# JoshuaQSH/FALCON-TTDforGNNs

Measured on AMD Instinct MI355X. Metric: tt_embedding_lookups_per_sec, higher is better.
Workload: dtype f32; 1 GPU; ogbn-products TTEmbeddingBag fwd+bwd+SGD per step, frontier of a 2048-seed batch = 409600 unique uniform ids per GPU, bag length 1; num_embeddings=2449029, ids_per_gpu_step=409600, parallelism=dp1

## Files before the change

### falcon-ttdforgnns_amd/csrc/ttemb_fast3.hip

```cpp
#include "ttemb_common.h"
#include "ttemb_cache.h"

#include <atomic>
#include <cstdlib>
#include <cstring>



namespace ttemb {

typedef float f32x4 __attribute__((ext_vector_type(4)));


constexpr int kChunk = 16;
constexpr uint32_t kMultiBit = 0x80000000u;

template <int Q0, int Q1, int Q2, int R1, int R2>
struct Cfg {
  static constexpr int M2 = Q0 * Q1;
  static constexpr int MT2 = (M2 + 15) / 16;
  static constexpr int KS1 = R1 / 4;
  static constexpr int KS2 = R2 / 4;
  static constexpr int N1 = Q1 * R2;
  static constexpr int NT1 = (N1 + 15) / 16;
  static constexpr int NT2 = Q2;
  static constexpr int D = Q0 * Q1 * Q2;
  static constexpr int ROW0 = Q0 * R1;
  static constexpr int ROW1 = R1 * Q1 * R2;
  static constexpr int ROW2 = R2 * Q2;
  static constexpr int LDA = R2 + 1;
  static constexpr int LDB = ROW2 + 4;
  static constexpr int LDO = D + 4;
  static constexpr int P_FLOATS = ((MT2 * 16 * LDA + 3) / 4) * 4;
  static constexpr int B_FLOATS = kChunk * LDB;
  static constexpr int O_FLOATS = kChunk * LDO;
  static constexpr int LDPB = (R2 % 32 == 0) ? R2 + 16 : R2;
  static constexpr int LDBB = (Q2 % 2 == 1 && ROW2 % 32 == 16) ? ROW2 : ROW2 + 4;
  static constexpr int BB2_FLOATS = kChunk * LDBB;
  static constexpr int DPAD = (M2 + 3) / 4 * 4 * Q2;
  static constexpr int LDOB = (((DPAD > D ? DPAD : D) + 15) / 32) * 32 + 16;
  static constexpr int OB_FLOATS = kChunk * LDOB;
  static constexpr int PB_FLOATS = ((M2 * LDPB + 3) / 4) * 4;
  static constexpr int BO_FLOATS = B_FLOATS > O_FLOATS ? B_FLOATS : O_FLOATS;
  static constexpr int WAVE_FLOATS = P_FLOATS + BO_FLOATS;
  static constexpr int RT1 = (R1 + 15) / 16;
  static constexpr int RT2 = (R2 + 15) / 16;
  static constexpr int LDG = N1 + 1;
  static constexpr int LD2 = ROW2 + 1;
  static constexpr int BB_FLOATS = B_FLOATS > P_FLOATS ? B_FLOATS : P_FLOATS;
  static constexpr int DB_FLOATS = ((O_FLOATS > R1 * LDG ? O_FLOATS : R1 * LDG) + 3) / 4 * 4;
  static constexpr int BWD_WAVE_FLOATS = P_FLOATS + BB_FLOATS + DB_FLOATS;
  static_assert(LDOB >= (M2 + 3) / 4 * 4 * Q2, "the padded K-step of the E product reads inside the staged row");
  static_assert(Q0 <= 16, "stage 1 pads q0 to one 16-row tile");
  static_assert(R1 % 4 == 0 && R2 % 4 == 0, "ranks must be multiples of the MFMA K");
  static_assert(N1 % 4 == 0, "rows of the prefix product move as float4");
  static_assert(D % 4 == 0 && ROW2 % 4 == 0, "rows move as float4");
  static_assert(ROW2 <= 256, "the dG2 reduce reads one E row per wavefront load");
};

typedef unsigned int u32x4 __attribute__((ext_vector_type(4)));
typedef __amdgpu_buffer_rsrc_t rsrc_t;
constexpr uint32_t kOob = 0xffffffffu;

__device__ __forceinline__ rsrc_t make_rsrc(const void* p, uint32_t bytes) {
  return __builtin_amdgcn_make_buffer_rsrc(const_cast<void*>(p), 0, (int)bytes, 0x00020000);
}
__device__ __forceinline__ float4 buf_load4(rsrc_t r, uint32_t voff) {
  const u32x4 v = __builtin_amdgcn_raw_buffer_load_b128(r, (int)voff, 0, 0);
  return make_float4(__uint_as_float(v.x), __uint_as_float(v.y), __uint_as_float(v.z), __uint_as_float(v.w));
}
__device__ __forceinline__ u32x4 buf_load4u(rsrc_t r, uint32_t voff) {
  return __builtin_amdgcn_raw_buffer_load_b128(r, (int)voff, 0, 0);
}
__device__ __forceinline__ uint32_t buf_load1u(rsrc_t r, uint32_t voff) {
  return __builtin_amdgcn_raw_buffer_load_b32(r, (int)voff, 0, 0);
}
__device__ __forceinline__ void buf_store4(rsrc_t r, uint32_t voff, const float4& x) {
  u32x4 v;
  v.x = __float_as_uint(x.x);
  v.y = __float_as_uint(x.y);
  v.z = __float_as_uint(x.z);
  v.w = __float_as_uint(x.w);
  __builtin_amdgcn_raw_buffer_store_b128(v, r, (int)voff, 0, 0);
}
#ifndef TTEMB_NT
#define TTEMB_NT 0
#endif
template <bool NT>
__device__ __forceinline__ void buf_store4_p(rsrc_t r, uint32_t voff, const float4& x) {
  u32x4 v;
  v.x = __float_as_uint(x.x);
  v.y = __float_as_uint(x.y);
  v.z = __float_as_uint(x.z);
  v.w = __float_as_uint(x.w);
  __builtin_amdgcn_raw_buffer_store_b128(v, r, (int)voff, 0, NT ? 2 : 0);
}
__device__ __forceinline__ void buf_store1(rsrc_t r, uint32_t voff, float x) {
  __builtin_amdgcn_raw_buffer_store_b32(__float_as_uint(x), r, (int)voff, 0, 0);
}

typedef const __attribute__((address_space(4))) uint32_t* desc_ptr;
__device__ __forceinline__ uint4 load_desc(desc_ptr tab, uint32_t c, uint32_t nchunks) {
  const uint32_t at = 4u * (c < nchunks ? c : (nchunks ? nchunks - 1 : 0u));
  const uint32_t keep = c < nchunks ? 0xffffffffu : 0u;
  return make_uint4(tab[at] & keep, tab[at + 1] & keep, tab[at + 2] & keep, tab[at + 3] & keep);
}

constexpr int kSortThreads = 1024;
#ifndef TTEMB_RANGE_THREADS
#define TTEMB_RANGE_THREADS 512
#endif
constexpr int kRangeThreads = TTEMB_RANGE_THREADS;
#ifndef TTEMB_SORT_SLICE
#define TTEMB_SORT_SLICE 2048
#endif
constexpr int kSliceIds = TTEMB_SORT_SLICE;
constexpr int kMaxSlices = 1024;
constexpr int kMaxRanges = 512;
constexpr int kSortBatch = 8;
constexpr uint32_t kFirstBit = 0x100u, kLastBit = 0x200u;
constexpr int kCountBanks = 8;
__host__ __device__ __forceinline__ uint64_t counter_tag(uint64_t epoch) { return ((epoch & ((1ull << 37) - 1ull)) | (1ull << 37)) << 26; }
constexpr int kOvfBits = 28;
constexpr uint64_t kOvfMask = (1ull << kOvfBits) - 1ull;
__host__ __device__ __forceinline__ uint64_t ovf_tag(uint64_t epoch) { return ((epoch & ((1ull << 35) - 1ull)) | (1ull << 35)) << kOvfBits; }
constexpr uint32_t kNoGroup = 0xffffffffu;
constexpr uint32_t kNoBlock = 0xffffffffu;
constexpr int kRoundIds = kSortThreads * 4;

struct Piece {
  long long pos0;
  long long count;
  long long rowbase;
  long long zero0, zero1;
  long long window_bytes;
};

struct GroupPlan {
  const Piece* piece;
  uint2* bucket;
  uint2* ovf;
  uint64_t* ovf_count;
  uint64_t* ovf_head;
  uint32_t cap;
  uint32_t banks;
  uint32_t ovf_slots;
  uint64_t* rcount;
  uint32_t* gstamp;
  uint64_t* epochs;
  uint64_t* rpub;
  uint32_t* i2s;
  uint32_t* vals;
  uint32_t* counts;
  uint64_t* gpre;
  uint4* ctab;
  float* ptab;
  float* etab;
  float* dptab;
  float* g2part;
  float* g0part;
  float* g1part;
  uint32_t* epi_live;
  uint32_t* wrows;
  uint32_t* wnrows;
  uint32_t* ticket;
  uint32_t use_ticket;
  uint32_t* fault_host;
  uint32_t spin_limit;
  uint32_t keep_p;
};

constexpr uint32_t kFaultTakeOver = 1u, kFaultLookBack = 2u, kFaultOverflow = 3u;
__device__ __forceinline__ uint64_t plan_tag(const GroupPlan& plan, uint64_t call) {
  const uint64_t salt = (reinterpret_cast<uint64_t>(plan.epochs) >> 8) * 0x9e3779b97f4a7c15ull;
  return (((call + salt) & ((1ull << 39) - 1ull)) | (1ull << 39)) << 24;
}
__device__ __forceinline__ void report_fault(const GroupPlan& plan, uint32_t G, uint64_t call, uint32_t code) {
  __hip_atomic_store(&plan.gpre[G + 2u], plan_tag(plan, call) | code, __ATOMIC_RELAXED, __HIP_MEMORY_SCOPE_AGENT);
  if (plan.fault_host != nullptr) __hip_atomic_store(plan.fault_host, code, __ATOMIC_RELAXED, __HIP_MEMORY_SCOPE_SYSTEM);
}
__device__ __forceinline__ bool plan_poisoned(const GroupPlan& plan, uint32_t G) {
  const desc_ptr w = (desc_ptr)plan.gpre;
  const uint32_t t_lo = w[2u * G + 2u], t_hi = w[2u * G + 3u], f_lo = w[2u * G + 4u], f_hi = w[2u * G + 5u];
  return t_hi == f_hi && ((t_lo ^ f_lo) >> 24) == 0u && (t_hi >> 31) != 0u;
}

__device__ __forceinline__ void poison_output(const GroupPlan& plan, float* out, uint32_t out_bytes, uint32_t row_floats, uint32_t gw,
                                              uint32_t nwaves, int lane) {
  if (plan.piece != nullptr) {
    out += plan.piece->rowbase * (long long)row_floats;
    out_bytes = (uint32_t)plan.piece->window_bytes;
  }
  const rsrc_t r = __builtin_amdgcn_make_buffer_rsrc(out, 0, (int)out_bytes, 0x00020000);
  const uint32_t qnan = 0x7fc00000u;
  u32x4 v;
  v.x = v.y = v.z = v.w = qnan;
  for (uint64_t off = ((uint64_t)gw * 64u + (uint32_t)lane) * 16u; off < out_bytes; off += (uint64_t)nwaves * 1024u)
    __builtin_amdgcn_raw_buffer_store_b128(v, r, (int)(uint32_t)off, 0, 0);
}

__device__ __forceinline__ uint64_t pack_count(uint32_t c) {
  return (uint64_t)c | ((uint64_t)((c + kChunk - 1) / kChunk) << 32);
}

template <typename T, int NT>
__device__ __forceinline__ T block_exclusive(T v, T* wave_sums, T& total) {
  const int lane = threadIdx.x & 63, wave = threadIdx.x >> 6;
  T incl = v;
#pragma unroll
  for (int d = 1; d < kWave; d <<= 1) {
    T up;
    if constexpr (sizeof(T) == 8) {
      const uint32_t lo_w = __shfl_up((uint32_t)incl, d, kWave), hi_w = __shfl_up((uint32_t)((uint64_t)incl >> 32), d, kWave);
      up = (T)((uint64_t)lo_w | ((uint64_t)hi_w << 32));
    } else {
      up = __shfl_up(incl, d, kWave);
    }
    if (lane >= d) incl += up;
  }
  if (lane == kWave - 1) wave_sums[wave] = incl;
  __syncthreads();
  T before = 0, all = 0;
  for (int w = 0; w < NT / kWave; ++w) {
    const T x = wave_sums[w];
    if (w < wave) before += x;
    all += x;
  }
  __syncthreads();
  total = all;
  return before + incl - v;
}

__device__ __forceinline__ uint64_t tagged_add(uint64_t* word, uint64_t tag, uint64_t mask, uint64_t v, uint32_t spin_limit,
                                               bool& taken) {
  unsigned long long* ctr = reinterpret_cast<unsigned long long*>(word);
  unsigned long long old = atomicAdd(ctr, (unsigned long long)v);
  taken = true;
  if ((old & ~mask) == tag) return old & mask;
  for (uint32_t tries = 0; tries < spin_limit; ++tries) {
    old = __hip_atomic_load(ctr, __ATOMIC_RELAXED, __HIP_MEMORY_SCOPE_AGENT);
    if ((old & ~mask) == tag) return atomicAdd(ctr, (unsigned long long)v) & mask;
    if (atomicCAS(ctr, old, tag | v) == old) return 0;
  }
  taken = false;
  return 0;
}

__global__ __launch_bounds__(kSortThreads) void fast3_decode_kernel(
    const int64_t* __restrict__ indices, const int64_t* __restrict__ rowidx,
    const int64_t* __restrict__ offsets, uint32_t nnz, uint32_t per_slice,
    const int32_t* __restrict__ nnz_dev, int64_t B, int D, float* __restrict__ zero_out, uint32_t sentinel,
    uint32_t p0, uint32_t p1, uint32_t p2, uint32_t shift, uint32_t ranges, GroupPlan plan) {
  __shared__ uint32_t hist[kMaxRanges];
  __shared__ uint32_t place[kMaxRanges];
  __shared__ uint32_t oslot[kMaxRanges];
  const uint64_t call = plan.epochs[0] + 1ull;
  const uint32_t epoch = (uint32_t)call;
  if (blockIdx.x == 0 && threadIdx.x == 0) {
    plan.epochs[1] = call;
    *plan.ticket = 0u;
  }
  const Piece* pc = plan.piece;
  const int64_t pos0 = pc ? pc->pos0 : 0, rowbase = pc ? pc->rowbase : 0;
  const int64_t cnt = pc ? pc->count : live_count(nnz, nnz_dev);
  const int64_t cnt_all = pos0 + cnt;
  const uint32_t s0 = blockIdx.x * per_slice;
  if (zero_out != nullptr) {
    const int64_t z0 = pc ? pc->zero0 : 0, z1 = pc ? pc->zero1 : B;
    const int64_t per_b = (z1 - z0 + gridDim.x - 1) / gridDim.x;
    const int64_t b1 = z0 + (blockIdx.x + 1) * per_b < z1 ? z0 + (blockIdx.x + 1) * per_b : z1;
    for (int64_t b = z0 + blockIdx.x * per_b + threadIdx.x; b < b1; b += kSortThreads)
      if (offsets[b + 1] - offsets[b] != 1) {
        float4* o = reinterpret_cast<float4*>(zero_out + b * D);
        for (int c = 0; c * 4 < D; ++c) o[c] = make_float4(0.f, 0.f, 0.f, 0.f);
      }
  }
  const uint32_t s1 = s0 + per_slice < nnz ? s0 + per_slice : nnz;
  const uint32_t bank = blockIdx.x % plan.banks, cap = plan.cap;
  const uint64_t tag = counter_tag(call), otag = ovf_tag(call);
  uint64_t* const rctr = plan.rcount + (size_t)bank * kMaxRanges;
  uint2* const bkt = plan.bucket + (size_t)bank * cap;
  const size_t rstride = (size_t)plan.banks * cap;
  constexpr int UD = kRoundIds / kSortThreads;
  for (uint32_t r0 = s0; r0 < s1; r0 += kRoundIds) {
    for (uint32_t i = threadIdx.x; i < ranges; i += kSortThreads) hist[i] = 0u;
    __syncthreads();
    int64_t idv[UD], o0[UD], o1[UD], rv[UD];
#pragma unroll
    for (int u = 0; u < UD; ++u) {
      const uint32_t n = r0 + threadIdx.x + u * kSortThreads;
      const int64_t g = pos0 + n;
      const bool on = n < s1 && (int64_t)n < cnt;
      idv[u] = on ? indices[g] : 0;
      rv[u] = on && rowidx != nullptr ? rowidx[g] : -1;
      const bool direct = on && rowidx == nullptr && g < B;
      o0[u] = direct ? offsets[g] : -1;
      o1[u] = direct ? offsets[g + 1] : -1;
    }
    uint32_t key[UD], val[UD], rng[UD], rank[UD];
#pragma unroll
    for (int u = 0; u < UD; ++u) {
      const uint32_t n = r0 + threadIdx.x + u * kSortThreads;
      rng[u] = kNoGroup;
      key[u] = val[u] = rank[u] = 0u;
      if (n >= s1 || (int64_t)n >= cnt) continue;
      int64_t id = idv[u];
      id = id < 0 ? 0 : (id >= (int64_t)sentinel ? (int64_t)sentinel - 1 : id);
      const int64_t g = pos0 + n;
      int64_t row;
      bool multi;
      if (rowidx != nullptr) {
        row = rv[u];
        multi = !bag_is_single(rowidx, offsets, g, cnt_all, row);
      } else if (o0[u] >= 0 && o0[u] <= g && g < o1[u]) {
        row = g;
        multi = o1[u] - o0[u] != 1;
      } else {
        int64_t lo = 0, hi = B;
        while (hi - lo > 1) {
          const int64_t mid = (lo + hi) >> 1;
          if (offsets[mid] <= g) lo = mid; else hi = mid;
        }
        row = lo;
        multi = offsets[row + 1] - offsets[row] != 1;
      }
      row -= rowbase;
      const uint32_t uu = (uint32_t)id;
      const uint32_t i0 = uu / (p1 * p2);
      const uint32_t rem = uu - i0 * (p1 * p2);
      const uint32_t i1 = rem / p2;
      const uint32_t group = i1 * p0 + i0;
      key[u] = (group & ((1u << shift) - 1u)) | ((rem - i1 * p2) << 16);
      val[u] = (uint32_t)row | (multi ? kMultiBit : 0u);
      rng[u] = group >> shift;
      plan.gstamp[group] = epoch;
      rank[u] = atomicAdd(&hist[rng[u]], 1u);
    }
    __syncthreads();
    for (uint32_t i = threadIdx.x; i < ranges; i += kSortThreads) {
      const uint32_t h = hist[i];
      uint32_t at = 0u, os = kNoBlock;
      if (h != 0u) {
        bool taken;
        at = (uint32_t)tagged_add(&rctr[i], tag, 0x3ffffffull, h, plan.spin_limit, taken);
        if (!taken) {
          report_fault(plan, p0 * p1, call, kFaultTakeOver);
          at = kNoBlock;
        } else if (at + h > cap) {
          const uint32_t len = at >= cap ? h : at + h - cap;
          const uint64_t b = tagged_add(plan.ovf_count, otag, kOvfMask, len + 1u, plan.spin_limit, taken);
          if (!taken) {
            report_fault(plan, p0 * p1, call, kFaultTakeOver);
            at = kNoBlock;
          } else if (b + 1u + len <= plan.ovf_slots) {
            const unsigned long long old = atomicExch(reinterpret_cast<unsigned long long*>(&plan.ovf_head[i]), otag | b);
            plan.ovf[b] = make_uint2(len, (old & ~kOvfMask) == otag ? (uint32_t)(old & kOvfMask) : kNoBlock);
            os = (uint32_t)b + 1u;
          } else {
            report_fault(plan, p0 * p1, call, kFaultOverflow);
            at = kNoBlock;
          }
        }
      }
      place[i] = at;
      oslot[i] = os;
    }
    __syncthreads();
#pragma unroll
    for (int u = 0; u < UD; ++u) {
      if (rng[u] == kNoGroup) continue;
      const uint32_t at = place[rng[u]];
      if (at == kNoBlock) continue;
      const uint32_t p = at + rank[u];
      if (p < cap) {
        bkt[rng[u] * rstride + p] = make_uint2(val[u], key[u]);
      } else {
        const uint32_t os = oslot[rng[u]];
        if (os != kNoBlock) plan.ovf[os + (p - (at > cap ? at : cap))] = make_uint2(val[u], key[u]);
      }
    }
    __syncthreads();
  }
}

template <typename F>
__device__ __forceinline__ void visit_range(const GroupPlan& plan, uint32_t range, const uint32_t* cum, uint32_t head,
                                            uint32_t nids, F&& f) {
  const uint2* bk = plan.bucket + (size_t)range * plan.banks * plan.cap;
  const uint32_t nb = cum[kCountBanks];
  for (uint32_t k0 = threadIdx.x; k0 < nb; k0 += kRangeThreads * kSortBatch) {
    uint2 e[kSortBatch];
#pragma unroll
    for (int u = 0; u < kSortBatch; ++u) {
      const uint32_t k = k0 + u * kRangeThreads;
      uint32_t b = 0;
#pragma unroll
      for (int j = 1; j < kCountBanks; ++j) b += k >= cum[j] ? 1u : 0u;
      e[u] = k < nb ? bk[(size_t)b * plan.cap + (k - cum[b])] : make_uint2(0u, kNoGroup);
    }
#pragma unroll
    for (int u = 0; u < kSortBatch; ++u) f(e[u]);
  }
  uint32_t blk = head;
  for (uint32_t hops = 0; blk != kNoBlock && hops < nids && blk < plan.ovf_slots; ++hops) {
    const uint2 h = plan.ovf[blk];
    const uint32_t len = h.x;
    if ((uint64_t)blk + 1u + len > plan.ovf_slots) break;
    for (uint32_t j = threadIdx.x; j < len; j += kRangeThreads) f(plan.ovf[blk + 1u + j]);
    blk = h.y;
  }
}

constexpr uint64_t kEpochMask = (1ull << 40) - 1ull;
static_assert(kMaxRanges <= kRangeThreads, "the look-back reads one published word per thread");
__device__ __forceinline__ void place_range(const uint32_t ranges, uint32_t G, uint32_t shift,
                                            uint32_t nnz, uint32_t max_chunks, const GroupPlan& plan, uint32_t* lds_s,
                                            uint64_t* red) {
  const uint32_t span = 1u << shift;
  uint32_t* cursor = lds_s;
  uint32_t* gfirst = cursor + span;
  uint32_t* gcount = gfirst + span;
  uint32_t* gchunk = gcount + span;
  constexpr int NWV = kRangeThreads / kWave;
  const uint64_t epoch = (plan.epochs[1] & (kEpochMask >> 1)) | (1ull << 39);
  const bool ticketed = plan.use_ticket != 0u;
  if (ticketed && threadIdx.x == 0) reinterpret_cast<uint32_t*>(red)[0] = atomicAdd(plan.ticket, 1u);
  for (uint32_t i = threadIdx.x; i < span; i += kRangeThreads) gcount[i] = 0u;
  __syncthreads();
  uint32_t range = blockIdx.x;
  if (ticketed) {
#ifdef TTEMB_TICKET_ROTATE
    range = (reinterpret_cast<uint32_t*>(red)[0] + 1u) % ranges;
#else
    range = reinterpret_cast<uint32_t*>(red)[0];
#endif
    if (range >= ranges) return;
  }
  const uint32_t g0 = range << shift;
  __shared__ uint32_t rinfo[kCountBanks + 3];
  {
    const uint64_t ctag = counter_tag(plan.epochs[1]);
    uint32_t c[kCountBanks], tot = 0u;
#pragma unroll
    for (int b = 0; b < kCountBanks; ++b) {
      const uint64_t w = threadIdx.x < ranges && (uint32_t)b < plan.banks ? plan.rcount[b * kMaxRanges + threadIdx.x] : 0ull;
      c[b] = (w & ~0x3ffffffull) == ctag ? (uint32_t)(w & 0x3ffffffull) : 0u;
      tot += c[b];
    }
    const uint64_t hw = threadIdx.x == 0 ? plan.ovf_head[range] : 0ull;
    __syncthreads();
    uint64_t all;
    const uint64_t excl = block_exclusive<uint64_t, kRangeThreads>(tot, red, all);
    if (threadIdx.x == range) {
      uint32_t acc = 0u;
#pragma unroll
      for (int b = 0; b < kCountBanks; ++b) {
        rinfo[b] = acc;
        acc += c[b] < plan.cap ? c[b] : plan.cap;
      }
      rinfo[kCountBanks] = acc;
      rinfo[kCountBanks + 1] = (uint32_t)excl;
    }
    if (threadIdx.x == 0) {
      const uint64_t otag = ovf_tag(plan.epochs[1]);
      rinfo[kCountBanks + 2] = (hw & ~kOvfMask) == otag ? (uint32_t)(hw & kOvfMask) : kNoBlock;
    }
    __syncthreads();
  }
  uint32_t cum[kCountBanks + 1];
#pragma unroll
  for (int b = 0; b <= kCountBanks; ++b) cum[b] = rinfo[b];
  const uint32_t n0 = rinfo[kCountBanks + 1], head = rinfo[kCountBanks + 2];
  const uint32_t nids = nnz;
  visit_range(plan, range, cum, head, nids, [&](uint2 e) {
    const uint32_t gl = e.y & 0xffffu;
    if (gl < span) atomicAdd(&gcount[gl], 1u);
  });
  __syncthreads();
  uint64_t carry = 0;
  uint32_t live_here = 0;
  for (uint32_t b0 = 0; b0 < span; b0 += kRangeThreads) {
    const uint32_t i = b0 + threadIdx.x;
    const bool on = i < span && g0 + i < G;
    const uint32_t c = i < span ? gcount[i] : 0u;
    uint64_t total;
    const uint64_t pre = carry + block_exclusive<uint64_t, kRangeThreads>(pack_count(c), red, total);
    if (i < span) {
      gfirst[i] = cursor[i] = n0 + (uint32_t)pre;
      gchunk[i] = (uint32_t)(pre >> 32);
    }
    if (on) plan.counts[g0 + i] = c;
    carry += total;
    live_here += (uint32_t)__syncthreads_count(c != 0u);
  }
  const uint32_t chunks_here = (uint32_t)(carry >> 32);
  const uint32_t n1 = n0 + (uint32_t)carry;
  if (threadIdx.x == 0) {
    __hip_atomic_store(&plan.rpub[range], (epoch << 24) | (uint64_t)chunks_here, __ATOMIC_RELAXED, __HIP_MEMORY_SCOPE_AGENT);
    __hip_atomic_store(&plan.rpub[ranges + range], (epoch << 24) | (uint64_t)live_here, __ATOMIC_RELAXED, __HIP_MEMORY_SCOPE_AGENT);
  }
  __syncthreads();
  visit_range(plan, range, cum, head, nids, [&](uint2 e) {
    const uint32_t gl = e.y & 0xffffu;
    if (gl >= span) return;
    const uint32_t dst = atomicAdd(&cursor[gl], 1u);
    if (dst >= nnz) return;
    plan.i2s[dst] = e.y >> 16;
    plan.vals[dst] = e.x;
  });
  uint64_t before = 0, live_before = 0;
  if (threadIdx.x < range) {
    const bool want_live = range == ranges - 1;
    uint64_t v = 0, w = epoch << 24;
    for (uint32_t spin = 0; spin < plan.spin_limit; ++spin) {
      v = __hip_atomic_load(&plan.rpub[threadIdx.x], __ATOMIC_RELAXED, __HIP_MEMORY_SCOPE_AGENT);
      if (want_live) w = __hip_atomic_load(&plan.rpub[ranges + threadIdx.x], __ATOMIC_RELAXED, __HIP_MEMORY_SCOPE_AGENT);
      if ((v >> 24) == epoch && (w >> 24) == epoch) break;
      __builtin_amdgcn_s_sleep(8);
    }
    const bool seen = (v >> 24) == epoch && (w >> 24) == epoch;
    before = seen ? (v & 0xffffffull) : 0ull;
    live_before = seen ? (w & 0xffffffull) : 0ull;
    if (!seen) report_fault(plan, G, plan.epochs[1], kFaultLookBack);
  }
#pragma unroll
  for (int d = kWave / 2; d > 0; d >>= 1) {
    before += __shfl_down((uint32_t)before, d, kWave);
    live_before += __shfl_down((uint32_t)live_before, d, kWave);
  }
  __syncthreads();
  if ((threadIdx.x & 63) == 0) {
    red[threadIdx.x >> 6] = before;
    red[NWV + 1 + (threadIdx.x >> 6)] = live_before;
  }
  __syncthreads();
  uint64_t chunk_base = 0, live_all = 0;
  for (int w = 0; w < NWV; ++w) {
    chunk_base += red[w];
    live_all += red[NWV + 1 + w];
  }
  for (uint32_t i = threadIdx.x; i < span; i += kRangeThreads) {
    const uint32_t g = g0 + i;
    if (g >= G) continue;
    const uint32_t c = gcount[i], first = gfirst[i];
    const uint32_t ch0 = (uint32_t)chunk_base + gchunk[i];
    plan.gpre[g] = (uint64_t)first | ((uint64_t)ch0 << 32);
    const uint32_t chunks = (c + kChunk - 1) / kChunk;
    for (uint32_t k = 0; k < chunks; ++k) {
      const uint32_t rest = c - k * kChunk;
      const uint32_t len = rest < (uint32_t)kChunk ? rest : (uint32_t)kChunk;
      if (ch0 + k < max_chunks)
        plan.ctab[ch0 + k] = make_uint4(first + k * kChunk, g, len | (k == 0 ? kFirstBit : 0u) | (k + 1 == chunks ? kLastBit : 0u), ch0 + chunks);
    }
  }
  if (threadIdx.x == 0) {
    if (range == ranges - 1) {
      plan.gpre[G] = (uint64_t)n1 | ((chunk_base + chunks_here) << 32);
      const uint64_t ptag = plan_tag(plan, plan.epochs[1]);
      plan.gpre[G + 1u] = ptag;
      unsigned long long* fw = reinterpret_cast<unsigned long long*>(&plan.gpre[G + 2u]);
      const unsigned long long seen = __hip_atomic_load(fw, __ATOMIC_RELAXED, __HIP_MEMORY_SCOPE_AGENT);
      if ((seen >> 24) != (ptag >> 24) && seen != 0ull) atomicCAS(fw, seen, 0ull);
      plan.counts[G] = (uint32_t)live_all + live_here;
    }
    if (range == 0) plan.epochs[0] = plan.epochs[1];
  }
  if (range == ranges - 1) {
    const uint64_t next = counter_tag(plan.epochs[1] + 1ull);
    for (uint32_t i = threadIdx.x; i < (uint32_t)kCountBanks * ranges; i += kRangeThreads)
      plan.rcount[(i / ranges) * kMaxRanges + i % ranges] = next;
    if (threadIdx.x == 0) *plan.ovf_count = ovf_tag(plan.epochs[1] + 1ull);
  }
}

__global__ __launch_bounds__(kRangeThreads) void fast3_place_kernel(uint32_t nnz, uint32_t max_chunks, uint32_t G, uint32_t shift,
                                                                    GroupPlan plan) {
  extern __shared__ uint32_t lds_s[];
  __shared__ uint64_t red[2 * (kRangeThreads / kWave + 1)];
  place_range(gridDim.x, G, shift, nnz, max_chunks, plan, lds_s, red);
}

__device__ __forceinline__ long long wave_bag_of_position(const int64_t* __restrict__ offsets, long long B, long long pos, int lane) {
  long long lo = 0, hi = B;
  while (hi - lo > 1) {
    const long long span = hi - lo, step = (span + kWave - 1) / kWave;
    long long probe = lo + (lane + 1) * step;
    probe = probe > hi ? hi : probe;
    const bool ok = probe < hi && (long long)offsets[probe] <= pos;
    const int k = __popcll(__ballot(ok));
    const long long nlo = k > 0 ? lo + k * step : lo;
    long long nhi = lo + (long long)(k + 1) * step;
    nhi = nhi > hi ? hi : nhi;
    lo = nlo;
    hi = nhi;
  }
  return lo;
}

__global__ __launch_bounds__(kWave) void plan_pieces_kernel(const int64_t* __restrict__ offsets, int64_t B, int64_t nnz,
                                                            const int32_t* __restrict__ nnz_dev, long long max_ids, long long max_rows,
                                                            int D, int slots, Piece* __restrict__ tab) {
  if (blockIdx.x != 0) return;
  const int lane = threadIdx.x;
  const long long total = live_count(nnz, nnz_dev);
  long long pos = 0, zr = 0;
  for (int k = 0; k < slots; ++k) {
    Piece pc;
    pc.pos0 = pos;
    pc.count = 0;
    pc.rowbase = 0;
    pc.zero0 = pc.zero1 = zr;
    pc.window_bytes = 0;
    if (pos < total) {
      const long long rb = wave_bag_of_position(offsets, B, pos, lane);
      const long long row_end = rb + max_rows;
      long long end = row_end < B ? (long long)offsets[row_end] : total;
      end = end > total ? total : end;
      end = end > pos + max_ids ? pos + max_ids : end;
      if (end <= pos) end = pos + 1;
      pc.count = end - pos;
      pc.rowbase = rb;
      if (end < total) {
        const long long nb = wave_bag_of_position(offsets, B, end, lane);
        pc.zero1 = (long long)offsets[nb] == end ? nb : nb + 1;
      } else {
        pc.zero1 = B;
      }
      if (pc.zero1 < pc.zero0) pc.zero1 = pc.zero0;
      const long long rows_left = B - rb < max_rows ? B - rb : max_rows;
      pc.window_bytes = rows_left * (long long)D * 4;
      zr = pc.zero1;
      pos = end;
    }
    if (lane == 0) tab[k] = pc;
  }
}

#ifndef TTEMB_PREFIX_GROUPS
#define TTEMB_PREFIX_GROUPS 8
#endif
constexpr int kPrefixGroups = TTEMB_PREFIX_GROUPS;
template <int Q0, int Q1, int Q2, int R1, int R2>
__device__ __forceinline__ void prefix_unit(const float* __restrict__ G0, const float* __restrict__ G1, uint32_t p0,
                                            const GroupPlan& plan, uint32_t i0_block, uint32_t i1, int lane, int stamps) {
  using C = Cfg<Q0, Q1, Q2, R1, R2>;
  constexpr int GM = 16 / Q0;
  const int hi = lane >> 4, lo = lane & 15;
  const uint32_t i0_begin = i0_block * kPrefixGroups;
  const uint32_t i0_end = i0_begin + kPrefixGroups < p0 ? i0_begin + kPrefixGroups : p0;
  const uint32_t my = i0_begin + lane;
  const uint32_t want = stamps == 0 ? 0u : (uint32_t)plan.epochs[1];
  const bool mine = lane < kPrefixGroups && my < i0_end &&
                    (stamps != 0 ? plan.gstamp[i1 * p0 + my] == want : plan.counts[i1 * p0 + my] != 0u);
  const unsigned long long live = __ballot(mine);
  if (!live) return;
  const float* g1 = G1 + (size_t)i1 * C::ROW1;
  float bv[C::KS1][C::NT1];
#pragma unroll
  for (int s = 0; s < C::KS1; ++s)
#pragma unroll
    for (int nt = 0; nt < C::NT1; ++nt)
      bv[s][nt] = (C::N1 % 16 == 0 || 16 * nt + lo < C::N1) ? g1[(4 * s + hi) * C::N1 + 16 * nt + lo] : 0.f;
  for (uint32_t base = 0; base < (uint32_t)kPrefixGroups; base += GM) {
    if (!((live >> base) & ((1ull << GM) - 1))) continue;
    const uint32_t i0a = i0_begin + base + lo / Q0;
    float av[C::KS1];
#pragma unroll
    for (int s = 0; s < C::KS1; ++s)
      av[s] = i0a < i0_end ? G0[(size_t)i0a * C::ROW0 + (lo % Q0) * R1 + 4 * s + hi] : 0.f;
    f32x4 acc[C::NT1];
#pragma unroll
    for (int nt = 0; nt < C::NT1; ++nt) {
      acc[nt] = (f32x4){0.f, 0.f, 0.f, 0.f};
#pragma unroll
      for (int s = 0; s < C::KS1; ++s) acc[nt] = __builtin_amdgcn_mfma_f32_16x16x4f32(av[s], bv[s][nt], acc[nt], 0, 0, 0);
    }
#pragma unroll
    for (int r = 0; r < 4; ++r) {
      const int row = 4 * hi + r;
      const uint32_t gi = base + row / Q0;
      const int a = row % Q0;
      if (row / Q0 >= GM || !((live >> gi) & 1ull)) continue;
      float* dst = plan.ptab + (size_t)(i1 * p0 + i0_begin + gi) * (C::M2 * R2);
#pragma unroll
      for (int nt = 0; nt < C::NT1; ++nt) {
        const int n = 16 * nt + lo;
        if (C::N1 % 16 == 0 || n < C::N1) dst[(a * Q1 + n / R2) * R2 + n % R2] = acc[nt][r];
      }
    }
  }
}

template <int Q0, int Q1, int Q2, int R1, int R2>
__global__ __launch_bounds__(64) void fast3_prefix_kernel(const float* __restrict__ G0, const float* __restrict__ G1,
                                                          uint32_t p0, uint32_t stamps, GroupPlan plan) {
  prefix_unit<Q0, Q1, Q2, R1, R2>(G0, G1, p0, plan, blockIdx.x, blockIdx.y, (int)threadIdx.x, (int)stamps);
}

template <int Q0, int Q1, int Q2, int R1, int R2>
__global__ __launch_bounds__(kRangeThreads) void fast3_place_prefix_kernel(uint32_t ranges, uint32_t nnz, uint32_t max_chunks,
                                                                          uint32_t G, uint32_t shift,
                                                                          const float* __restrict__ G0,
                                                                          const float* __restrict__ G1, uint32_t p0,
                                                                          uint32_t p1, GroupPlan plan) {
  extern __shared__ uint32_t lds_s[];
  __shared__ uint64_t red[2 * (kRangeThreads / kWave + 1)];
  if (blockIdx.x < ranges) {
    place_range(ranges, G, shift, nnz, max_chunks, plan, lds_s, red);
    return;
  }
  const uint32_t blocks0 = (p0 + kPrefixGroups - 1) / kPrefixGroups;
  const uint32_t unit = (blockIdx.x - ranges) * (kRangeThreads / kWave) + (threadIdx.x >> 6);
  if (unit >= blocks0 * p1) return;
  prefix_unit<Q0, Q1, Q2, R1, R2>(G0, G1, p0, plan, unit % blocks0, unit / blocks0, (int)(threadIdx.x & 63), 1);
}

#ifndef TTEMB_CHAIN_WAVES
#define TTEMB_CHAIN_WAVES 4
#endif
constexpr int kChainWaves = TTEMB_CHAIN_WAVES;
constexpr uint32_t kOobBase = 0x80000000u;

__device__ __forceinline__ uint32_t uniform(uint32_t x) { return __builtin_amdgcn_readfirstlane(x); }
#ifdef TTEMB_NO_PRIO
#define TTEMB_PRIO(x)
#else
#define TTEMB_PRIO(x) __builtin_amdgcn_s_setprio(x)
#endif

template <int Q0, int Q1, int Q2, int R1, int R2>
__global__ __launch_bounds__(kChainWaves * 64) void fast3_forward_kernel(const float* __restrict__ G2, GroupPlan plan, uint32_t G,
                                                                         uint32_t p2, uint32_t nnz, float* __restrict__ out,
                                                                         uint32_t out_bytes) {
  using C = Cfg<Q0, Q1, Q2, R1, R2>;
  extern __shared__ __attribute__((aligned(16))) float smem[];
  const int lane = threadIdx.x & 63;
  const uint32_t wave = uniform(threadIdx.x >> 6);
  const int hi = lane >> 4, lo = lane & 15;
  const int b_l = lane >> 2, j_l = lane & 3;
  float* pbuf = smem + wave * C::WAVE_FLOATS;
  float* bbuf = pbuf + C::P_FLOATS;
  float* obuf = bbuf;

  const desc_ptr ctab = (desc_ptr)plan.ctab;
  const uint32_t nchunks = ((desc_ptr)plan.gpre)[2u * G + 1u];
  const uint32_t nwaves = gridDim.x * kChainWaves, gw = blockIdx.x * kChainWaves + wave;
  if (plan_poisoned(plan, G)) {
    poison_output(plan, out, out_bytes, (uint32_t)C::D, gw, nwaves, lane);
    return;
  }
  const uint32_t per = (nchunks + nwaves - 1) / nwaves;
  const uint32_t c0 = gw * per;
  if (c0 >= nchunks) return;
  const uint32_t c1 = c0 + per < nchunks ? c0 + per : nchunks;

  constexpr int F4G = C::ROW2 / 4, NLG = (F4G + 3) / 4;
  constexpr int D4 = C::D / 4, NLO = (D4 + 3) / 4;
  constexpr int PF = C::M2 * R2, PF4 = PF / 4, NLP = (PF4 + kWave - 1) / kWave;
  const rsrc_t r_g2 = make_rsrc(G2, p2 * (uint32_t)C::ROW2 * 4u);
  if (plan.piece != nullptr) {
    out += plan.piece->rowbase * (long long)C::D;
    out_bytes = (uint32_t)plan.piece->window_bytes;
  }
  const rsrc_t r_out = make_rsrc(out, out_bytes);
  const uint32_t rowpiece = 16u * (uint32_t)j_l;
  const uint32_t g_last = (F4G % 4 == 0 || j_l + 4 * (NLG - 1) < F4G) ? rowpiece + 64u * (NLG - 1) : kOobBase;
  const bool o_has_last = D4 % 4 == 0 || j_l + 4 * (NLO - 1) < D4;

  float4 pre_g[NLG], pre_p[NLP];
  auto request = [&](uint32_t row, const uint4& d) {
#pragma unroll
    for (int k = 0; k < NLG; ++k)
      pre_g[k] = k + 1 < NLG ? buf_load4(r_g2, row + rowpiece + 64u * k) : buf_load4(r_g2, row + g_last);
    const rsrc_t r_p = make_rsrc(plan.ptab + (size_t)uniform(d.y) * PF, uniform((d.z & kFirstBit) ? (uint32_t)(PF * 4) : 0u));
#pragma unroll
    for (int it = 0; it < NLP; ++it) pre_p[it] = buf_load4(r_p, 16u * (uint32_t)lane + 1024u * it);
  };
  auto stage = [&](bool with_p) {
    if (with_p) {
#pragma unroll
      for (int it = 0; it < NLP; ++it) {
        const int e = it * kWave + lane;
        if (PF4 % kWave == 0 || e < PF4) {
          float* dst = pbuf + (4 * e / R2) * C::LDA + (4 * e) % R2;
          dst[0] = pre_p[it].x;
          dst[1] = pre_p[it].y;
          dst[2] = pre_p[it].z;
          dst[3] = pre_p[it].w;
        }
      }
    }
#pragma unroll
    for (int k = 0; k < NLG; ++k) {
      const int idx = j_l + 4 * k;
      if (F4G % 4 == 0 || idx < F4G) *reinterpret_cast<float4*>(bbuf + b_l * C::LDB + 4 * idx) = pre_g[k];
    }
  };

  auto fetch_i2 = [&](const uint4& d) {
    return buf_load1u(make_rsrc(plan.i2s + uniform(d.x), uniform((d.z & 0xffu) * 4u)), 4u * (uint32_t)b_l);
  };
  auto fetch_val = [&](const uint4& d) {
    return buf_load1u(make_rsrc(plan.vals + uniform(d.x), uniform((d.z & 0xffu) * 4u)), 4u * (uint32_t)b_l);
  };
  uint4 d_cur = load_desc(ctab, c0, c1);
  uint4 d_nxt = load_desc(ctab, c0 + 1, c1);
  uint4 d_nn = load_desc(ctab, c0 + 2, c1);
  uint4 d_n3 = load_desc(ctab, c0 + 3, c1);
  uint32_t i2_nn, val_cur;
  {
#if defined(TTEMB_ABL) && (TTEMB_ABL & 256)
    const uint32_t i2_a = (uint32_t)b_l, i2_b = (uint32_t)b_l + 16u;
// ... 2734 lines not shown
```

Baseline: 2.176 billion lookups/s.

## Fuse bag zeroing into grouping loop and keep bucket entries in registers

Two changes to the grouping kernels. First, in the direct-offsets case, zeroing of multi-element bag outputs now happens inside the main id loop, reusing offsets already loaded, with a tail pass for bags beyond the live count. This replaces a separate pre-pass that re-read offsets. Second, when a range's bucket capacity fits in the threads times batch size, place_range loads its bucket entries into registers once and reuses them for both the counting pass and the placement pass, instead of reading the buckets twice from global memory. The cost is more register use, and the behavior is gated by a compile-time trips mask.

```diff
diff --git a/falcon-ttdforgnns_amd/csrc/ttemb_fast3.hip b/falcon-ttdforgnns_amd/csrc/ttemb_fast3.hip
--- a/falcon-ttdforgnns_amd/csrc/ttemb_fast3.hip
+++ b/falcon-ttdforgnns_amd/csrc/ttemb_fast3.hip
@@ -127,6 +127,10 @@
 constexpr uint32_t kNoGroup = 0xffffffffu;
 constexpr uint32_t kNoBlock = 0xffffffffu;
 constexpr int kRoundIds = kSortThreads * 4;
+#ifndef TTEMB_GROUPING_TRIPS
+#define TTEMB_GROUPING_TRIPS 9
+#endif
+constexpr bool kTripClear = (TTEMB_GROUPING_TRIPS & 1) != 0, kTripOneVisit = (TTEMB_GROUPING_TRIPS & 8) != 0;
 
 struct Piece {
   long long pos0;
@@ -265,8 +269,7 @@
   const int64_t cnt = pc ? pc->count : live_count(nnz, nnz_dev);
   const int64_t cnt_all = pos0 + cnt;
   const uint32_t s0 = blockIdx.x * per_slice;
-  if (zero_out != nullptr) {
-    const int64_t z0 = pc ? pc->zero0 : 0, z1 = pc ? pc->zero1 : B;
+  auto clear_bags = [&](int64_t z0, int64_t z1) {
     const int64_t per_b = (z1 - z0 + gridDim.x - 1) / gridDim.x;
     const int64_t b1 = z0 + (blockIdx.x + 1) * per_b < z1 ? z0 + (blockIdx.x + 1) * per_b : z1;
     for (int64_t b = z0 + blockIdx.x * per_b + threadIdx.x; b < b1; b += kSortThreads)
@@ -274,7 +277,9 @@
         float4* o = reinterpret_cast<float4*>(zero_out + b * D);
         for (int c = 0; c * 4 < D; ++c) o[c] = make_float4(0.f, 0.f, 0.f, 0.f);
       }
-  }
+  };
+  const bool clear_here = kTripClear && zero_out != nullptr && rowidx == nullptr && pc == nullptr;
+  if (zero_out != nullptr && !clear_here) clear_bags(pc ? pc->zero0 : 0, pc ? pc->zero1 : B);
   const uint32_t s1 = s0 + per_slice < nnz ? s0 + per_slice : nnz;
   const uint32_t bank = blockIdx.x % plan.banks, cap = plan.cap;
   const uint64_t tag = counter_tag(call), otag = ovf_tag(call);
@@ -307,6 +312,10 @@
       int64_t id = idv[u];
       id = id < 0 ? 0 : (id >= (int64_t)sentinel ? (int64_t)sentinel - 1 : id);
       const int64_t g = pos0 + n;
+      if (clear_here && g < B && o1[u] - o0[u] != 1) {
+        float4* o = reinterpret_cast<float4*>(zero_out + g * D);
+        for (int c = 0; c * 4 < D; ++c) o[c] = make_float4(0.f, 0.f, 0.f, 0.f);
+      }
       int64_t row;
       bool multi;
       if (rowidx != nullptr) {
@@ -381,8 +390,23 @@
     }
     __syncthreads();
   }
-}
-
+  if (clear_here) {
+    const int64_t zb = cnt < B ? (cnt < 0 ? 0 : cnt) : B;
+    if (zb < B) clear_bags(zb, B);
+  }
+}
+
+template <typename F>
+__device__ __forceinline__ void visit_overflow(const GroupPlan& plan, uint32_t head, uint32_t nids, F&& f) {
+  uint32_t blk = head;
+  for (uint32_t hops = 0; blk != kNoBlock && hops < nids && blk < plan.ovf_slots; ++hops) {
+    const uint2 h = plan.ovf[blk];
+    const uint32_t len = h.x;
+    if ((uint64_t)blk + 1u + len > plan.ovf_slots) break;
+    for (uint32_t j = threadIdx.x; j < len; j += kRangeThreads) f(plan.ovf[blk + 1u + j]);
+    blk = h.y;
+  }
+}
 template <typename F>
 __device__ __forceinline__ void visit_range(const GroupPlan& plan, uint32_t range, const uint32_t* cum, uint32_t head,
                                             uint32_t nids, F&& f) {
@@ -401,14 +425,7 @@
 #pragma unroll
     for (int u = 0; u < kSortBatch; ++u) f(e[u]);
   }
-  uint32_t blk = head;
-  for (uint32_t hops = 0; blk != kNoBlock && hops < nids && blk < plan.ovf_slots; ++hops) {
-    const uint2 h = plan.ovf[blk];
-    const uint32_t len = h.x;
-    if ((uint64_t)blk + 1u + len > plan.ovf_slots) break;
-    for (uint32_t j = threadIdx.x; j < len; j += kRangeThreads) f(plan.ovf[blk + 1u + j]);
-    blk = h.y;
-  }
+  visit_overflow(plan, head, nids, f);
 }
 
 constexpr uint64_t kEpochMask = (1ull << 40) - 1ull;
@@ -472,10 +489,33 @@
   for (int b = 0; b <= kCountBanks; ++b) cum[b] = rinfo[b];
   const uint32_t n0 = rinfo[kCountBanks + 1], head = rinfo[kCountBanks + 2];
   const uint32_t nids = nnz;
-  visit_range(plan, range, cum, head, nids, [&](uint2 e) {
-    const uint32_t gl = e.y & 0xffffu;
+  const uint2* const bk = plan.bucket + (size_t)range * plan.banks * plan.cap;
+  const bool held = kTripOneVisit && (uint64_t)plan.banks * plan.cap <= (uint64_t)kRangeThreads * kSortBatch;
+  uint2 e[kSortBatch];
+#pragma unroll
+  for (int u = 0; u < kSortBatch; ++u) e[u] = make_uint2(0u, kNoGroup);
+  if (held && cum[kCountBanks] != 0u) {
+#pragma unroll
+    for (int u = 0; u < kSortBatch; ++u) {
+      const uint32_t k = threadIdx.x + u * kRangeThreads;
+      uint32_t b = 0;
+#pragma unroll
+      for (int j = 1; j < kCountBanks; ++j) b += k >= cum[j] ? 1u : 0u;
+      const uint2 w = bk[k < cum[kCountBanks] ? (size_t)b * plan.cap + (k - cum[b]) : (size_t)0];
+      if (k < cum[kCountBanks]) e[u] = w;
+    }
+  }
+  auto count_entry = [&](uint2 w) {
+    const uint32_t gl = w.y & 0xffffu;
     if (gl < span) atomicAdd(&gcount[gl], 1u);
-  });
+  };
+  if (held) {
+#pragma unroll
+    for (int u = 0; u < kSortBatch; ++u) count_entry(e[u]);
+    visit_overflow(plan, head, nids, count_entry);
+  } else {
+    visit_range(plan, range, cum, head, nids, count_entry);
+  }
   __syncthreads();
   uint64_t carry = 0;
   uint32_t live_here = 0;
@@ -500,14 +540,21 @@
     __hip_atomic_store(&plan.rpub[ranges + range], (epoch << 24) | (uint64_t)live_here, __ATOMIC_RELAXED, __HIP_MEMORY_SCOPE_AGENT);
   }
   __syncthreads();
-  visit_range(plan, range, cum, head, nids, [&](uint2 e) {
-    const uint32_t gl = e.y & 0xffffu;
+  auto place_entry = [&](uint2 w) {
+    const uint32_t gl = w.y & 0xffffu;
     if (gl >= span) return;
     const uint32_t dst = atomicAdd(&cursor[gl], 1u);
     if (dst >= nnz) return;
-    plan.i2s[dst] = e.y >> 16;
-    plan.vals[dst] = e.x;
-  });
+    plan.i2s[dst] = w.y >> 16;
+    plan.vals[dst] = w.x;
+  };
+  if (held) {
+#pragma unroll
+    for (int u = 0; u < kSortBatch; ++u) place_entry(e[u]);
+    visit_overflow(plan, head, nids, place_entry);
+  } else {
+    visit_range(plan, range, cum, head, nids, place_entry);
+  }
   uint64_t before = 0, live_before = 0;
   if (threadIdx.x < range) {
     const bool want_live = range == ranges - 1;
```

After: 2.165 billion lookups/s. No clear change (-0.5%).
